# eridgd/WCT-TF

Measured on AMD Instinct MI355X. Metric: stylized frames/sec @512x512, 5-level relu5->1 pipeline, alpha=0.8, higher is better.
Workload: dtype f16

## Files before the change

wct_tf_amd/build.py:

```python
import hashlib
import os
import subprocess
import sys
from concurrent.futures import ThreadPoolExecutor

HERE = os.path.dirname(os.path.abspath(__file__))
CSRC = os.path.join(HERE, 'csrc')
LIB = os.path.join(HERE, 'libwct_hip.so')
WCT_UNITS = ['stats_gemm.hip', 'eigh.hip', 'spectral.hip', 'wct.hip', 'mask.hip', 'style_swap.hip', 'warm.hip']
API_UNITS = ['api_ctx.hip', 'api_weights.hip', 'api_drivers.hip', 'api_ops.hip', 'api_stylize.hip', 'api_train.hip']
SOURCES = API_UNITS + ['conv.hip', 'conv_wino.hip', 'coral.hip', 'colors.hip', 'guided.hip', 'guided_color.hip', 'guided_time.hip', 'guided_motion.hip', 'noise.hip', 'resize.hip', 'banded.hip', 'wrap.hip', 'train.hip'] + WCT_UNITS


STAMP = LIB + '.src.sha256'
FLAGS = ['--offload-arch=gfx950', '-O3', '-std=c++17', '-fPIC', '-Wno-unused-value', '-Wno-unused-result']
FILE_FLAGS = {u: ['-fno-slp-vectorize'] for u in WCT_UNITS}


def source_digest():
    h = hashlib.sha256((' '.join(FLAGS) + repr(sorted(FILE_FLAGS.items()))).encode())
    deps = sorted(os.path.join(CSRC, f) for f in os.listdir(CSRC) if f.endswith(('.hip', '.h')))
    deps.append(os.path.join(os.path.dirname(HERE), 'include', 'wct_hip.h'))
    for d in deps:
        h.update(os.path.basename(d).encode())
# ... 37 lines not shown
```

wct_tf_amd/csrc/banded.hip:

```cpp
#include "api.h"
#include "wct_stages.h"
#include "pool_rule.h"

static const int BAND_RE[6] = {0, 16, 16, 16, 48, 96};
static const int BAND_RD[6] = {0, 2, 2, 3, 4, 5};
constexpr int BAND_ROWS_CAP = 2048;
constexpr size_t LAUNCH_BYTES = WCT_LAUNCH_BYTES;

struct Band { int e0, e1, y0, y1, d0, d1, f0, f1; };

static void band_list(int H, int level, int band_rows, std::vector<Band>* out) {
  const int s = 1 << (level - 1), h = (H + s - 1) / s, Re = BAND_RE[level], Rd = BAND_RD[level];
  out->clear();
  for (long long y = 0; y < H; y += band_rows) {
    Band b;
    b.y0 = (int)y; b.y1 = (int)std::min<long long>(H, y + band_rows);
    b.e0 = std::max(0, b.y0 - Re); b.e1 = (int)std::min<long long>(H, (long long)b.y1 + Re);
    b.f0 = b.y0 / s; b.f1 = b.y1 == H ? h : b.y1 / s;
    b.d0 = std::max(0, b.f0 - Rd) & ~1; b.d1 = std::min(h, b.f1 + Rd);
    out->push_back(b);
  }
}

static bool enc_fits(long long rows, long long W, int level) {
// ... 334 lines not shown
      HIP_TRY(hipGetLastError());
      HIP_TRY(hipMemcpyAsync(cp.means + (size_t)k0 * C, gp.w.mean, (size_t)G * C * sizeof(float), hipMemcpyDeviceToDevice, s));
      HIP_TRY(hipMemcpyAsync(cp.scales + k0, gp.w.scale, (size_t)G * sizeof(float), hipMemcpyDeviceToDevice, s));
    }
    hipLaunchKernelGGL(pool_finish_kernel, dim3(C), dim3(C), 0, s, (const double*)cp.acc, (const float*)cp.means, (const float*)cp.scales,
                       (const int*)cp.n, K, C, cov_eps(mode, r.eps), w.mean, w.A, w.A0, w.scale);
    HIP_TRY(hipGetLastError());
  }
  if ((stages & WCT_STAGE_EIG) && (rc = launch_eig_stage(w, C, 1, cp.tail.skip, 1, r.sweeps_dev, r.eig_fail, s))) return rc;
  if (!(stages & WCT_STAGE_APPLY)) return WCT_OK;
  if (prep) {
    WctStyleSlots slots = {};
    slots.state[0] = prep->state[0];
    if ((rc = launch_style_load_slots(slots, 1, w, C, true, s))) return rc;
  }
  if ((rc = launch_spectral_tail(w, C, 1, r.alpha, mode, r.eps, cp.tail.skip, 1, s))) return rc;
  if ((rc = launch_blend(w, C, 1, r.alpha, cp.tail.skip, s))) return rc;
  for (int k = 0; k < K; ++k) {
    const size_t at = (size_t)k * n_full * C;
    if ((rc = launch_apply(w, content + at, k == K - 1 ? n_last : n_full, C, 1, r.out16 ? r.out16 + at : nullptr, r.out32 ? r.out32 + at : nullptr, s)))
      return rc;
  }
  return WCT_OK;
}

int run_transform_chunked(wct_ctx* c, const float* fc, size_t Nc, int n_full, int K, const float* fs, int Ns, int C, float alpha,
                          unsigned flags, float eps, half_t* out16, float* out32, int* sweeps_dev, const WctStyleRef* prep) {
  ARG_CHECK(K >= 1 && n_full >= 1 && Nc > (size_t)n_full * (K - 1) && Nc < LAUNCH_BYTES);
  if (flags & WCT_FLAG_ADAIN) { wct_set_error("a chunked transform is a whiten-colour transform: WCT_FLAG_ADAIN is not served"); return WCT_ERR_ARG; }
  if (K == 1) return run_transform(c, fc, (int)Nc, fs, Ns, C, 1, alpha, flags, eps, out16, out32, sweeps_dev, nullptr, prep);
  if (K > CHUNKS_MAX) { wct_set_error("%d chunks: at most %d per map", K, CHUNKS_MAX); return WCT_ERR_ARG; }
// ... 12 lines not shown
```

wct_tf_amd/csrc/mask.hip:

```cpp
#include "wct_stages.h"
#include <algorithm>
#include <type_traits>

constexpr int MASK_ROWS = 2048;
constexpr int SEG_STRIDE = WCT_MIX_MAX + 1;

__device__ __forceinline__ int mask_label(const MaskGeom& g, int r) {
  const int i = r / g.w, j = r - i * g.w;
  return g.mask[(size_t)min(i * g.stride, g.Hm - 1) * g.Wm + min(j * g.stride, g.Wm - 1)];
}

__global__ __launch_bounds__(256) void mask_count_kernel(MaskGeom g, int N, int K, int* counts) {
  __shared__ int wc[4][WCT_MIX_MAX];
  g.mask += (size_t)blockIdx.y * g.Hm * g.Wm;
  counts += (size_t)blockIdx.y * gridDim.x * WCT_MIX_MAX;
  const int lane = threadIdx.x & 63, wave = threadIdx.x >> 6;
  int cnt[WCT_MIX_MAX];
#pragma unroll
  for (int k = 0; k < WCT_MIX_MAX; ++k) cnt[k] = 0;
  const int base = blockIdx.x * MASK_ROWS;
  for (int it = 0; it < MASK_ROWS / 256; ++it) {
    const int r = base + it * 256 + threadIdx.x;
    const int lab = r < N ? mask_label(g, r) : -1;
#pragma unroll
// ... 217 lines not shown
  const int mode = r.mode, stages = r.stages; hipStream_t s = r.stream;
  MaskPlan m;
  ARG_CHECK(C % 32 == 0 && C >= 32 && C <= 1024 && content && styles && mask_plan(&m, r.workspace, C, Nc, nk, styles, Ns, K, 2));
  ARG_CHECK(mode == WCT_MODE_NP || mode == WCT_MODE_TF);
  ARG_CHECK(launch_map_fits((size_t)Nc * C, 4) && plan_fits(m, C));
  ARG_CHECK(r.workspace_bytes >= m.total);
  const WctCarve& w = m.w;
  int rc;
  if (stages & WCT_STAGE_COV) {
    if ((rc = launch_mask_gather(content, g, Nc, K, C, m, 1, s))) return rc;
    if ((rc = launch_plan_stats(m, C, false, true, cov_eps(mode, r.eps), s))) return rc;
  }
  if ((stages & WCT_STAGE_EIG) && m.P > 0 && (rc = launch_eig_stage(w, C, m.P, m.skip, 1, r.sweeps_dev, r.eig_fail, s))) return rc;
  if (!(stages & WCT_STAGE_APPLY)) return WCT_OK;
  if (m.P > 0) {
    if ((rc = launch_spectral_tail(w, C, m.P, r.alpha, mode, r.eps, m.skip, m.nwhite, s))) return rc;
    if ((rc = launch_blend(w, C, m.P, r.alpha, m.skip, s))) return rc;
    ApplySegArgs a = apply_args<ApplySegArgs>(w, m.xg, 0, C, r.out16, r.out32);
    a.seg_off = m.seg_off; a.perm = m.perm;
    for (int p = 0; p < WCT_MIX_MAX; ++p) a.lab[p] = m.lab[p];
    if ((rc = launch_apply_args(a, m.nmax, m.P, s))) return rc;
  }
  return launch_mask_passthrough(content, Nc, C, m, 1, K, r.out16, r.out32, s);
}

struct SegLabels { int lab[WCT_MIX_MAX]; };
struct SegBatchLabels { unsigned char fl[WCT_PLAN_PAIRS]; int N; };
template <typename Labels>
__global__ void adain_seg_apply_kernel(const float* xg, const int* seg_off, const int* perm, Labels sl, int C, const float* mean,
                                       const float* var, float alpha, float eps, half_t* out16, float* out32) {
  const int pair = blockIdx.y;
// ... 116 lines not shown
  ARG_CHECK(C % 32 == 0 && C >= 32 && C <= 1024 && content && mask_batch_plan(&m, r.workspace, C, Nc, G, nk, Ns, K, 2));
  ARG_CHECK(mode == WCT_MODE_NP || mode == WCT_MODE_TF);
  ARG_CHECK(launch_map_fits((size_t)Nc * C, 4) && plan_fits(m, C));
  ARG_CHECK((size_t)G * Nc < ((size_t)1 << 31));
  ARG_CHECK(r.workspace_bytes >= m.total);
  const WctCarve& w = m.w;
  int rc;
  if (stages & WCT_STAGE_COV) {
    if ((rc = launch_mask_gather(content, g, Nc, K, C, m, m.G, s))) return rc;
    if ((rc = launch_plan_stats(m, C, false, true, cov_eps(mode, r.eps), s))) return rc;
  }
  if ((stages & WCT_STAGE_EIG) && m.P > 0 && (rc = launch_eig_stage(w, C, m.P, m.skip, 1, nullptr, r.eig_fail, s))) return rc;
  if (!(stages & WCT_STAGE_APPLY)) return WCT_OK;
  if (m.P > 0) {
    if ((rc = launch_style_load_slots(states, m.P, w, C, true, s))) return rc;
    if ((rc = launch_spectral_tail(w, C, m.P, r.alpha, mode, r.eps, m.skip, m.nwhite, s))) return rc;
    if ((rc = launch_blend(w, C, m.P, r.alpha, m.skip, s))) return rc;
    ApplySegBatchArgs a = apply_args<ApplySegBatchArgs>(w, m.xg, Nc, C, r.out16, r.out32);
    a.seg_off = m.seg_off; a.perm = m.perm;
    for (int p = 0; p < WCT_PLAN_PAIRS; ++p) a.fl[p] = m.fl[p];
    if ((rc = launch_apply_args(a, m.nmax, m.P, s))) return rc;
  }
  return launch_mask_passthrough(content, Nc, C, m, m.G, K, r.out16, r.out32, s);
}

int launch_adain_masked_batch(const float* content, int Nc, int G, const MaskGeom& g, const int* nk, const int* Ns, int K, int C,
                              const WctCall& r, const WctStyleSlots& states) {
  hipStream_t s = r.stream;
  MaskBatchPlan m;
  ARG_CHECK(C % 32 == 0 && C <= 1024 && content && mask_batch_plan(&m, r.workspace, C, Nc, G, nk, Ns, K, 1));
  ARG_CHECK((size_t)G * Nc < ((size_t)1 << 31));
// ... 18 lines not shown
```

wct_tf_amd/csrc/spectral.hip:

```cpp
#include "wct_stages.h"

__device__ __forceinline__ bool pair_resolved(float dp, float dq, float e) { return e * e <= 0.25f * dp * dq; }

constexpr float SPECTRAL_NOISE_CUT = 2.f;
__device__ __forceinline__ float spectral_cut(const float* Am, int C, int tid, float* red) {
  float mn = 0.f;
  for (int i = tid; i < C; i += 256) mn = fminf(mn, Am[(size_t)i * C + i]);
  for (int o = 32; o > 0; o >>= 1) mn = fminf(mn, __shfl_xor(mn, o, 64));
  if ((tid & 63) == 0) red[tid >> 6] = mn;
  __syncthreads();
  mn = fminf(fminf(red[0], red[1]), fminf(red[2], red[3]));
  return fmaxf(1e-5f, -SPECTRAL_NOISE_CUT * mn);
}

__device__ __forceinline__ float spectral_entry(float dp, float dq, float e, bool diag, int kind, float shift, float cut) {
  const bool kp = dp > cut, kq = dq > cut;
  if (diag) return kp ? (kind == 0 ? 1.f / sqrtf(dp + shift) : sqrtf(dp + shift)) : 0.f;
  if (!kp && !kq) return 0.f;
  if (kp && kq) {
    if (!pair_resolved(dp, dq, e)) return 0.f;
    const float sa = sqrtf(dp + shift), sb = sqrtf(dq + shift);
    return kind == 0 ? -e / (sa * sb * (sa + sb)) : e / (sa + sb);
  }
  const float dk = kp ? dp : dq, dd = kp ? dq : dp;
// ... 13 lines not shown
  for (int i = 0; i < 4; ++i) {
    const int r = q0 + ty * 4 + i, c = p0 + tx * 4;
    f32x4 v = {0.f, 0.f, 0.f, 0.f};
    if (r < C && c < C) v = *reinterpret_cast<const f32x4*>(Am + (size_t)r * C + c);
#pragma unroll
    for (int j = 0; j < 4; ++j) t.mt[ty * 4 + i][tx * 4 + j] = v[j];
  }
}

struct SpecAllArgs {
  const float* A;
  float* G;
  float *N, *R, *Pm;
  const float *X1, *X2;
  int C; float shift; int correct, second; WctSkip skip;
  unsigned* mabs; const float* mean; float* bias; float alpha; int mode;
};

__global__ __launch_bounds__(256) void spectral_open_all_kernel(SpecAllArgs a) {
  __shared__ SpectralTile t;
  const int m = blockIdx.z, p0 = blockIdx.y * 64, q0 = blockIdx.x * 64, tid = threadIdx.x;
  const int C = a.C, kind = m & 1, pair = m >> 1;
  const size_t cc = (size_t)C * C;
  if (kind == 0 && blockIdx.x == 0 && blockIdx.y == 0) {
    if (tid == 0) a.mabs[pair] = 0u;
    const float* mp = a.mean + (size_t)(one_content(a.skip) ? 0 : pair) * 2 * C;
    const float* ms = a.mean + (size_t)(one_style(a.skip) ? 0 : pair) * 2 * C + C;
    for (int i = tid; i < C; i += 256) {
      float b = a.alpha * ms[i];
      if (a.mode == WCT_MODE_TF) b += (1.f - a.alpha) * mp[i];
      a.bias[pair * C + i] = b;
    }
// ... 14 lines not shown
    f32x4 g, n4 = {0.f, 0.f, 0.f, 0.f}, r4 = n4, p4 = n4;
#pragma unroll
    for (int j = 0; j < 4; ++j) {
      const float dk = t.dq[tx * 4 + j];
      const float em = 0.5f * (av[j] + t.mt[tx * 4 + j][pl]);
      g[j] = spectral_entry(dp, dk, a.correct ? em : 0.f, p == q + j, kind, a.shift, cut);
      if (a.second && p != q + j && dp > cut && dk > cut && pair_resolved(dp, dk, em)) {
        const float sp = sqrtf(dp + a.shift), sk = sqrtf(dk + a.shift);
        n4[j] = em / (sp + sk);
        r4[j] = em / sk;
        p4[j] = n4[j] / sk;
      }
    }
    const size_t o = (size_t)p * C + q;
    *reinterpret_cast<f32x4*>(a.G + m * cc + o) = g;
    if (a.second) {
      *reinterpret_cast<f32x4*>(a.N + m * cc + o) = n4;
      if (kind == 0) { *reinterpret_cast<f32x4*>(a.R + pair * cc + o) = r4; *reinterpret_cast<f32x4*>(a.Pm + pair * cc + o) = p4; }
    }
  }
}

__global__ __launch_bounds__(256) void spectral_add2_all_kernel(SpecAllArgs a) {
  __shared__ float dps[64], dqs[64];
  __shared__ float x1t[64][65], x2t[64][65];
  const int m = blockIdx.z, p0 = blockIdx.y * 64, q0 = blockIdx.x * 64, tid = threadIdx.x;
  if (skip_style_mat(m, a.skip)) return;
  const int C = a.C, kind = m & 1;
  const size_t cc = (size_t)C * C;
  const float* Am = a.A + m * cc;
  float* Gm = a.G + m * cc;
  const float* X2 = a.X2 + m * cc;
  const float* X1 = a.X1 + (size_t)(m >> 1) * cc;
  int near = 0;
  for (int i = tid; i < C; i += 256) {
    const float d = fabsf(Am[(size_t)i * C + i]);
    near |= (d > 3.3e-6f) & (d < 3e-5f);
  }
  if (__syncthreads_or(near)) return;
  __shared__ float cutred[4];
  const float cut = spectral_cut(Am, C, tid, cutred);
  if (tid < 64) dps[tid] = p0 + tid < C ? Am[(size_t)(p0 + tid) * C + p0 + tid] : 0.f;
  else if (tid < 128) dqs[tid - 64] = q0 + tid - 64 < C ? Am[(size_t)(q0 + tid - 64) * C + q0 + tid - 64] : 0.f;
  const int ty = tid >> 4, tx = tid & 15;
#pragma unroll
  for (int i = 0; i < 4; ++i) {
    const int r = q0 + ty * 4 + i, c = p0 + tx * 4;
    f32x4 v1 = {0.f, 0.f, 0.f, 0.f}, v2 = v1;
    if (r < C && c < C) {
      v2 = *reinterpret_cast<const f32x4*>(X2 + (size_t)r * C + c);
      if (kind == 0) v1 = *reinterpret_cast<const f32x4*>(X1 + (size_t)r * C + c);
    }
#pragma unroll
    for (int j = 0; j < 4; ++j) { x2t[ty * 4 + i][tx * 4 + j] = v2[j]; x1t[ty * 4 + i][tx * 4 + j] = v1[j]; }
  }
  __syncthreads();
#pragma unroll
  for (int i = 0; i < 4; ++i) {
    const int pl = ty * 4 + i, p = p0 + pl, q = q0 + tx * 4;
    if (p >= C || q >= C) continue;
    const size_t o = (size_t)p * C + q;
    const f32x4 x2 = *reinterpret_cast<const f32x4*>(X2 + o);
    f32x4 x1 = {0.f, 0.f, 0.f, 0.f};
    if (kind == 0) x1 = *reinterpret_cast<const f32x4*>(X1 + o);
    f32x4 g = *reinterpret_cast<const f32x4*>(Gm + o);
    const float dp = dps[pl];
#pragma unroll
    for (int j = 0; j < 4; ++j) {
      const float dq = dqs[tx * 4 + j];
      if (!(dp > cut && dq > cut)) continue;
      const float sp = sqrtf(dp + a.shift), sq = sqrtf(dq + a.shift);
      float l2;
      if (kind == 1) l2 = -0.5f * (x2[j] + x2t[tx * 4 + j][pl]) / (sp + sq);
      else l2 = (0.5f * (x1[j] + x1t[tx * 4 + j][pl]) + 0.25f * (sp + sq) * (x2[j] + x2t[tx * 4 + j][pl])) / (sp * sq * (sp + sq));
      g[j] += l2;
    }
    *reinterpret_cast<f32x4*>(Gm + o) = g;
  }
}

static GemmArgs level_product(int C, WctSkip skip) {
  GemmArgs g = {};
  g.lda = g.ldb = g.ldo = C; g.M = g.N = g.K = g.ksplit = C; g.sA = g.sB = g.s_out = (size_t)C * C; g.skip = skip;
  return g;
}

static int launch_refresh(const WctCarve& w, int C, int P, WctSkip skip, hipStream_t s) {
  int rc;
  GemmArgs r1 = level_product(C, skip);
  r1.A = w.A0; r1.a_kmajor = 0; r1.B = w.V; r1.b_kmajor = 1; r1.out32 = w.X;
  r1.mask_diag = w.A; r1.s_mask = (size_t)C * C; r1.mask_out = w.refresh;
  if ((rc = launch_gemm(r1, 1, 2 * P, s))) return rc;
  GemmArgs r2 = level_product(C, skip);
  r2.A = w.V; r2.a_kmajor = 1; r2.B = w.X; r2.b_kmajor = 1; r2.out32 = w.A; r2.mask_in = w.refresh;
  return launch_gemm(r2, 1, 2 * P, s);
}

int launch_spectral_tail_refreshed(const WctCarve& w, int C, int P, float alpha, int mode, float eps_in, WctSkip skip, int nwhite,
                                   hipStream_t s) {
  int rc;
  const size_t cc = (size_t)C * C;
  const float shift = mode == WCT_MODE_NP ? (eps_in >= 0.f ? eps_in : 1e-5f) : 0.f;
  const int second = EIG_CORRECT >= 2;
  const dim3 tiles(cdiv(C, 64), cdiv(C, 64), 2 * P);
  SpecAllArgs sa = {};
  sa.A = w.A; sa.G = w.G; sa.C = C; sa.shift = shift; sa.correct = EIG_CORRECT; sa.second = second; sa.skip = skip;
  sa.N = w.S2; float* X2 = sa.N + 2 * P * cc; sa.R = X2 + 2 * P * cc; sa.Pm = sa.R + P * cc; float* X1 = sa.Pm + P * cc;
  sa.X1 = X1; sa.X2 = X2;
  sa.mabs = w.mabs; sa.mean = w.mean; sa.bias = w.bias; sa.alpha = alpha; sa.mode = mode;
  hipLaunchKernelGGL(spectral_open_all_kernel, tiles, dim3(256), 0, s, sa);
  HIP_TRY(hipGetLastError());
  if (second) {
    GemmArgs a = level_product(C, skip);
    a.A = sa.Pm; a.A_odd = sa.N + cc; a.sA_odd = 2 * cc; a.a_kmajor = 0; a.B = sa.N; a.b_kmajor = 1; a.out32 = X2;
    if ((rc = launch_gemm(a, 1, 2 * P, s))) return rc;
    GemmArgs b = level_product(C, WCT_SKIP_NONE);
    b.A = sa.R; b.a_kmajor = 0; b.B = sa.N; b.b_kmajor = 1; b.sB = 2 * cc; b.out32 = X1;
    if (nwhite > 0 && (rc = launch_gemm(b, 1, nwhite, s))) return rc;
    hipLaunchKernelGGL(spectral_add2_all_kernel, tiles, dim3(256), 0, s, sa);
    HIP_TRY(hipGetLastError());
  }
  GemmArgs g = level_product(C, skip);
  g.A = w.V; g.a_kmajor = 0; g.B = w.G; g.b_kmajor = 1; g.out32 = w.X;
  if ((rc = launch_gemm(g, 1, 2 * P, s))) return rc;
  GemmArgs h = level_product(C, skip);
  h.A = w.X; h.a_kmajor = 0; h.B = w.V; h.b_kmajor = 0; h.out32 = w.Tw;
  return launch_gemm(h, 1, 2 * P, s);
}

int launch_spectral_tail(const WctCarve& w, int C, int P, float alpha, int mode, float eps_in, WctSkip skip, int nwhite,
                         hipStream_t s) {
  const int rc = launch_refresh(w, C, P, skip, s);
  return rc ? rc : launch_spectral_tail_refreshed(w, C, P, alpha, mode, eps_in, skip, nwhite, s);
}
```

wct_tf_amd/csrc/style_swap.hip:

```cpp
#include "wct_stages.h"

__global__ void im2col_kernel(const float* src, float* dst, int w, int C, int p, int st, int ho, int wo) {
  const int c4n = C / 4;
  const size_t total = (size_t)ho * wo * p * p * c4n;
  for (size_t e = blockIdx.x * (size_t)blockDim.x + threadIdx.x; e < total; e += (size_t)gridDim.x * blockDim.x) {
    const int c4 = (int)(e % c4n);
    size_t t = e / c4n;
    const int j = (int)(t % p); t /= p;
    const int i = (int)(t % p); t /= p;
    const int x = (int)(t % wo), y = (int)(t / wo);
    reinterpret_cast<f32x4*>(dst)[e] =
        *reinterpret_cast<const f32x4*>(src + ((size_t)(y * st + i) * w + (x * st + j)) * C + c4 * 4);
  }
}

__global__ void patch_axis_inv_norm_kernel(const float* B, float* inv, int n, int K) {
  const int k4 = blockIdx.x * blockDim.x + threadIdx.x;
  if (k4 * 4 >= K) return;
  f32x4 s = {0.f, 0.f, 0.f, 0.f};
  for (int r = 0; r < n; ++r) {
    const f32x4 v = *reinterpret_cast<const f32x4*>(B + (size_t)r * K + k4 * 4);
    s += v * v;
  }
  f32x4 o;
// ... 111 lines not shown
                  "(swap_filter_fit / center_crop_to, wct.py:84-90)", patch, stride, hc, wc,
                  (ho - 1) * stride + patch, (wo - 1) * stride + patch);
    return WCT_ERR_ARG;
  }
  const int Nc = hc * wc, Ns = hs * ws, Mo = ho * wo, Pn = rows * cols, K = patch * patch * C;
  const size_t wct_bytes = align_up(wct_workspace_bytes(C, Nc, Ns, 1));
  ARG_CHECK(workspace_bytes >= style_swap_workspace_bytes(C, hc, wc, hs, ws, patch, stride));
  WctCarve w = carve(workspace, C, 1, pair_layout(C, Nc, Ns));
  SwapCarve sw = swap_carve((char*)workspace + wct_bytes, C, hc, wc, hs, ws, patch, stride);
  int rc;
  WctCall r = {};
  r.alpha = alpha; r.mode = WCT_MODE_TF; r.eps = eps; r.workspace = workspace; r.workspace_bytes = wct_bytes;
  r.stages = WCT_STAGE_COV | WCT_STAGE_EIG | WCT_STAGE_EIG_FP32UPDATE; r.eig_fail = eig_fail; r.stream = s;
  if ((rc = launch_wct(content, Nc, style, Ns, C, 1, WCT_SKIP_NONE, r, nullptr, nullptr, nullptr))) return rc;
  const size_t cc = (size_t)C * C;
  if ((rc = launch_spectral_tail(w, C, 1, alpha, WCT_MODE_TF, eps, WCT_SKIP_NONE, 1, s))) return rc;
  WctCarve v = w;
  v.A += cc; v.V += cc; v.G += cc; v.X += cc; v.Tw = w.T;
  if ((rc = launch_spectral_tail_refreshed(v, C, 1, alpha, WCT_MODE_TF, eps, WCT_SKIP_STYLE, 1, s))) return rc;
  auto apply = [&](const float* X, int N, const float* mean, const float* T, float* out) {
    GemmArgs g = {};
    g.A = X; g.lda = C; g.a_kmajor = 0; g.a_sub_k = mean; g.B = T; g.ldb = C; g.b_kmajor = 0;
    g.M = N; g.N = C; g.K = C; g.ksplit = C; g.out32 = out; g.ldo = C;
    return launch_gemm(g, 1, 1, s);
  };
  if ((rc = apply(content, Nc, w.mean, w.Tw, sw.Wc))) return rc;
  if ((rc = apply(style, Ns, w.mean + C, w.T, sw.Ws))) return rc;
  hipLaunchKernelGGL(im2col_kernel, dim3(ew_grid((size_t)Mo * K / 4)), dim3(256), 0, s, sw.Wc, sw.Ac, wc, C, patch, stride, ho, wo);
  hipLaunchKernelGGL(im2col_kernel, dim3(ew_grid((size_t)Pn * K / 4)), dim3(256), 0, s, sw.Ws, sw.Bs, ws, C, patch, stride, rows, cols);
  hipLaunchKernelGGL(patch_axis_inv_norm_kernel, dim3(cdiv(K / 4, 64)), dim3(64), 0, s, sw.Bs, sw.inv, Pn, K);
  HIP_TRY(hipGetLastError());
  {
    GemmArgs g = {};
    g.A = sw.Ac; g.lda = K; g.a_kmajor = 0; g.a_scale_k = sw.inv; g.B = sw.Bs; g.ldb = K; g.b_kmajor = 0;
// ... 20 lines not shown
```

wct_tf_amd/csrc/wct.hip:

```cpp
#include "wct_stages.h"
#include "jacobi_dev.h"
#include "strength_rule.h"
#include "conv_first_tile.h"
#include <algorithm>
#include <type_traits>



template <int BC, int BP, typename Args = ApplyArgs>
__global__ __launch_bounds__(256, 2) void apply_f16x2_kernel(Args p) {
  constexpr bool SEGB = std::is_same<Args, ApplySegBatchArgs>::value;
  constexpr bool SEG = std::is_same<Args, ApplySegArgs>::value || SEGB;
  constexpr bool MAP = std::is_same<Args, ApplyMapArgs>::value;
  constexpr int TM = BC / 64, TN = BP / 64;
  constexpr int MI = BC * 4 / 256, XI = BP * 4 / 256;
  __shared__ __attribute__((aligned(16))) unsigned char lm[2][BC * 64];
  __shared__ __attribute__((aligned(16))) unsigned char lx[2][BP * 64];
  typedef unsigned int u32x4 __attribute__((ext_vector_type(4)));
  const int tid = threadIdx.x, lane = tid & 63, wave = tid >> 6;
  const int wm = wave >> 1, wn = wave & 1;
  const int pair = blockIdx.z;
  const int n0 = blockIdx.x * BP, c0 = blockIdx.y * BC;
  int seg0 = 0, N = p.N;
  [[maybe_unused]] int row0 = 0;
// ... 511 lines not shown
  ARG_CHECK(style && state && C % 32 == 0 && C >= 32 && C <= 1024 && Ns >= (adain ? 1 : 2) && launch_map_fits((size_t)Ns * C, 4));
  ARG_CHECK(adain || mode == WCT_MODE_NP || mode == WCT_MODE_TF);
  ARG_CHECK(key.nslab >= 1 && key.nslab <= 256 && key.nsplit >= 1 && key.ksplit >= 256 && key.ksplit % 32 == 0 &&
            (long long)key.nsplit * key.ksplit >= Ns);
  SlotPlan sp;
  style_plan(&sp, r.workspace, C, style, Ns, key);
  ARG_CHECK(r.workspace_bytes >= sp.total);
  const WctCarve& w = sp.w;
  int rc;
  if (adain) {
    if ((rc = launch_plan_stats(sp, C, true, false, 0.f, s))) return rc;
    HIP_TRY(hipMemcpyAsync(state + C, w.var + C, (size_t)C * sizeof(float), hipMemcpyDeviceToDevice, s));
  } else {
    if ((rc = launch_plan_stats(sp, C, false, true, cov_eps(mode, r.eps), s))) return rc;
    if ((rc = launch_eig_stage(w, C, sp.P, sp.skip, 1, nullptr, r.eig_fail, s))) return rc;
    if ((rc = launch_spectral_tail(w, C, sp.P, 1.f, mode, r.eps, sp.skip, sp.nwhite, s))) return rc;
    HIP_TRY(hipMemcpyAsync(state + 2 * C, w.Tw + (size_t)C * C, (size_t)C * C * sizeof(float), hipMemcpyDeviceToDevice, s));
  }
  HIP_TRY(hipMemcpyAsync(state, w.mean + C, (size_t)C * sizeof(float), hipMemcpyDeviceToDevice, s));
  return WCT_OK;
}

int launch_wct(const float* content, int Nc, const float* style, int Ns, int C, int P, WctSkip skip, const WctCall& r,
               const WctFeatStats* stats, const WctStyleRef* prep, const WctWarmRef* warm, const WctStrength* sm, const WctImageSrc* src) {
  const int mode = r.mode, stages = r.stages; hipStream_t s = r.stream;
  ARG_CHECK(C % 32 == 0 && C >= 32 && C <= 1024 && Nc >= 2 && Ns >= 2 && P >= 1 && P <= 32);
  ARG_CHECK(!src || (C == 64 && !prep && !warm && !sm && stats && stats->u[0] && stats->umax[0] && stats->u[1] && stats->umax[1] &&
                     src->side[0].H * src->side[0].W == Nc && src->side[1].H * src->side[1].W == Ns));
  ARG_CHECK(!sm || strength_ok(*sm, Nc));
  ARG_CHECK(skip == WCT_SKIP_NONE || skip == WCT_SKIP_SHARED_STYLE);
  ARG_CHECK(!warm || (warm->basis && (skip == WCT_SKIP_NONE || prep)));
// ... 8 lines not shown
    if (src) rc = launch_cov_image(*src, P, w, cov_eps(mode, r.eps), skip, s);
    else rc = launch_cov(content, Nc, style, Ns, C, P, w, cov_eps(mode, r.eps), skip, s);
    if (rc) return rc;
  }
  if (stages & WCT_STAGE_EIG) {
    const bool rotate = warm && warm->valid;
    if (rotate && (rc = launch_warm_rotate(w, C, P, warm->basis, s))) return rc;
    if ((rc = launch_eig_stage(w, C, P, skip, (stages & WCT_STAGE_EIG_FP32UPDATE) ? 0 : 1, r.sweeps_dev, r.eig_fail, s, rotate ? 0 : 2)))
      return rc;
    if (rotate && (rc = launch_warm_compose(w, C, P, warm->basis, s))) return rc;
    if (warm && (rc = launch_warm_store(w.V + (size_t)2 * (P - 1) * C * C, w.X, warm->basis, C, s))) return rc;
  }
  if (!(stages & WCT_STAGE_APPLY)) return WCT_OK;

  if (prep && (rc = launch_style_load(*prep, 1, w, C, true, s))) return rc;
  if ((rc = launch_spectral_tail(w, C, P, sm ? 1.f : r.alpha, mode, r.eps, skip, P, s))) return rc;
  if (sm) return launch_blend_apply_map(w, content, Nc, C, P, skip, r, *sm);
  if (src) {
    if ((rc = launch_blend(w, C, P, r.alpha, skip, s))) return rc;
    return launch_apply_image(w, *src, P, r.out16, r.out32, s);
  }
  return launch_blend_apply(w, content, Nc, C, P, skip, r);
}

void plan_carve(SlotPlan* sp, void* base, int C) {
  PairLayout mx = {1, 1, 0};
  for (int m = 0; m < 2 * sp->P; ++m)
    if (sp->slot[m].n) { mx.nslab = std::max(mx.nslab, sp->slot[m].lay.nslab); mx.nsplit = std::max(mx.nsplit, sp->slot[m].lay.nsplit); }
  sp->w = carve(base, C, std::max(sp->P, 1), mx);
  sp->total = sp->w.total;
}
// ... 55 lines not shown
int launch_wct_mix(const float* content, int Nc, const float* const* styles, const int* Ns, int K, const float* lambda, int C,
                   const WctCall& r, const WctFeatStats* stats, const WctStyleRef* prep) {
  const int mode = r.mode, stages = r.stages; hipStream_t s = r.stream;
  SlotPlan sp;
  ARG_CHECK(C % 32 == 0 && C >= 32 && C <= 1024 && Nc >= 2 && content && (styles || prep) &&
            mix_plan(&sp, r.workspace, C, content, Nc, prep ? nullptr : styles, Ns, K, lambda, 2, stats, prep != nullptr));
  ARG_CHECK(mode == WCT_MODE_NP || mode == WCT_MODE_TF);
  ARG_CHECK(plan_fits(sp, C));
  ARG_CHECK(r.workspace_bytes >= sp.total);
  const WctCarve& w = sp.w;
  int rc;
  if ((stages & WCT_STAGE_COV) && (rc = launch_plan_stats(sp, C, false, true, cov_eps(mode, r.eps), s))) return rc;
  if ((stages & WCT_STAGE_EIG) && (rc = launch_eig_stage(w, C, sp.P, sp.skip, 1, r.sweeps_dev, r.eig_fail, s))) return rc;
  if (!(stages & WCT_STAGE_APPLY)) return WCT_OK;
  if (prep && (rc = launch_style_load(*prep, K, w, C, true, s))) return rc;
  if ((rc = launch_spectral_tail(w, C, sp.P, r.alpha, mode, r.eps, sp.skip, sp.nwhite, s))) return rc;
  MixWeights mw = {};
  mw.K = K;
  for (int k = 0; k < K; ++k) mw.lambda[k] = lambda[k];
  const size_t n4 = (size_t)C * C / 4;
  hipLaunchKernelGGL(wct_mix_kernel, dim3((unsigned)std::min<size_t>((n4 + 255) / 256, 1024)), dim3(256), 0, s, w.Tw, w.bias, C, mw);
  HIP_TRY(hipGetLastError());
  return launch_blend_apply(w, content, Nc, C, 1, WCT_SKIP_NONE, r);
}

__global__ void adain_apply_kernel(const float* x, size_t n4_per_pair, int C, const float* mean, const float* var,
                                   float alpha, float eps, half_t* out16, float* out32, int style_of_pair0,
                                   const float* mix_mu = nullptr, const float* mix_sd = nullptr) {
  const int pair = blockIdx.y;
  const int cq = C / 4;
  const float* mp = mean + (size_t)pair * 2 * C;
// ... 116 lines not shown
```

wct_tf_amd/csrc/wct_stages.h:

```cpp
#pragma once
#include "common.h"


constexpr int EIG_CORRECT = 2;
constexpr float JACOBI_TOL_FN = 1.5e-2f;
constexpr float JACOBI_TOL_FN2 = 4e-2f;
constexpr float JACOBI_TOL_FN_WCT = EIG_CORRECT >= 2 ? JACOBI_TOL_FN2 : (EIG_CORRECT ? JACOBI_TOL_FN : 0.f);

static inline size_t align_up(size_t x) { return (x + 255) & ~(size_t)255; }

struct WctCarve {
  float *mean, *var, *stat_partial, *absmax, *scale, *cov_partial, *A, *A0, *V, *d, *G, *X, *S2, *Tw, *Tcs, *T, *M, *bias, *mix;
  unsigned* mabs; int* refresh;
  void* jacobi_ws; size_t jacobi_bytes;
  int nslab, nsplit, ksplit;
  size_t total;
};

struct PairLayout { int nslab, nsplit, ksplit; };
PairLayout pair_layout(int C, int Nc, int Ns);
WctCarve carve(void* base, int C, int P, const PairLayout& lay);

static inline float cov_eps(int mode, float eps_in) {
  return mode == WCT_MODE_TF ? (eps_in >= 0.f ? eps_in : 1e-8f) : 0.f;
// ... 32 lines not shown
  a.x = x; a.N = N; a.C = C; a.mean = w.mean; a.M = w.M; a.bias = w.bias;
  a.xscale = w.scale; a.mabs = w.mabs; a.out16 = out16; a.out32 = out32;
  return a;
}
__device__ __host__ __forceinline__ int seg_frame(unsigned char fl) { return fl >> 3; }
__device__ __host__ __forceinline__ int seg_label(unsigned char fl) { return fl & 7; }

int launch_means(const float* content, int Nc, const float* style, int Ns, int C, int P, const WctCarve& w, bool with_var,
                 WctSkip skip, hipStream_t s, const WctFeatStats* fs);
int launch_cov(const float* content, int Nc, const float* style, int Ns, int C, int P, const WctCarve& w, float eps, WctSkip skip,
               hipStream_t s);
int launch_plan_stats(const SlotPlan& sp, int C, bool with_var, bool with_cov, float eps, hipStream_t s);
int launch_cov_image(const WctImageSrc& src, int P, const WctCarve& w, float eps, WctSkip skip, hipStream_t s);
int launch_eig_stage(const WctCarve& w, int C, int P, WctSkip skip, int u_f16, int* sweeps_dev, int* eig_fail, hipStream_t s,
                     int check_from = 2);
int launch_spectral_tail(const WctCarve& w, int C, int P, float alpha, int mode, float eps_in, WctSkip skip, int nwhite, hipStream_t s);
int launch_spectral_tail_refreshed(const WctCarve& w, int C, int P, float alpha, int mode, float eps_in, WctSkip skip, int nwhite,
                                   hipStream_t s);
int launch_blend(const WctCarve& w, int C, int P, float alpha, WctSkip skip, hipStream_t s);
int launch_apply(const WctCarve& w, const float* content, int Nc, int C, int P, half_t* out16, float* out32, hipStream_t s);
template <typename Args> int launch_apply_args(const Args& a, int nmax, int P, hipStream_t s);
int launch_warm_rotate(const WctCarve& w, int C, int P, const float* V0, hipStream_t s);
int launch_warm_compose(const WctCarve& w, int C, int P, const float* V0, hipStream_t s);
int launch_warm_store(const float* V, float* scratch, float* basis, int C, hipStream_t s);
int launch_style_load_slots(const WctStyleSlots& r, int P, const WctCarve& w, int C, bool with_T, hipStream_t s);
```

Before: 698.3.

## Run second-order spectral products as split-bf16 MFMA GEMMs with upper-triangle tiles

In the spectral tail, the second-order correction matrices are stored as hi/lo bf16 planes and multiplied by a new MFMA kernel that uses three bf16 products to approximate fp32 accuracy. The symmetric X2 product computes only upper-triangular tiles, and the add kernel reads the mirrored half to reconstruct the full matrix. This is meant to replace the fp32 GEMM path with cheaper matrix-core work and roughly halve the symmetric product. It costs some precision and adds a new kernel, and it is enabled by default with an environment variable to fall back to fp32.

```diff
diff --git a/wct_tf_amd/build.py b/wct_tf_amd/build.py
--- a/wct_tf_amd/build.py
+++ b/wct_tf_amd/build.py
@@ -7,7 +7,7 @@
 HERE = os.path.dirname(os.path.abspath(__file__))
 CSRC = os.path.join(HERE, 'csrc')
 LIB = os.path.join(HERE, 'libwct_hip.so')
-WCT_UNITS = ['stats_gemm.hip', 'eigh.hip', 'spectral.hip', 'wct.hip', 'mask.hip', 'style_swap.hip', 'warm.hip']
+WCT_UNITS = ['stats_gemm.hip', 'eigh.hip', 'spectral.hip', 'spectral_gemm.hip', 'wct.hip', 'mask.hip', 'style_swap.hip', 'warm.hip']
 API_UNITS = ['api_ctx.hip', 'api_weights.hip', 'api_drivers.hip', 'api_ops.hip', 'api_stylize.hip', 'api_train.hip']
 SOURCES = API_UNITS + ['conv.hip', 'conv_wino.hip', 'coral.hip', 'colors.hip', 'guided.hip', 'guided_color.hip', 'guided_time.hip', 'guided_motion.hip', 'noise.hip', 'resize.hip', 'banded.hip', 'wrap.hip', 'train.hip'] + WCT_UNITS
 
diff --git a/wct_tf_amd/csrc/banded.hip b/wct_tf_amd/csrc/banded.hip
--- a/wct_tf_amd/csrc/banded.hip
+++ b/wct_tf_amd/csrc/banded.hip
@@ -372,7 +372,7 @@
     slots.state[0] = prep->state[0];
     if ((rc = launch_style_load_slots(slots, 1, w, C, true, s))) return rc;
   }
-  if ((rc = launch_spectral_tail(w, C, 1, r.alpha, mode, r.eps, cp.tail.skip, 1, s))) return rc;
+  if ((rc = launch_spectral_tail(w, C, 1, r.alpha, mode, r.eps, cp.tail.skip, 1, second_order_bf16(), s))) return rc;
   if ((rc = launch_blend(w, C, 1, r.alpha, cp.tail.skip, s))) return rc;
   for (int k = 0; k < K; ++k) {
     const size_t at = (size_t)k * n_full * C;
diff --git a/wct_tf_amd/csrc/mask.hip b/wct_tf_amd/csrc/mask.hip
--- a/wct_tf_amd/csrc/mask.hip
+++ b/wct_tf_amd/csrc/mask.hip
@@ -255,7 +255,7 @@
   if ((stages & WCT_STAGE_EIG) && m.P > 0 && (rc = launch_eig_stage(w, C, m.P, m.skip, 1, r.sweeps_dev, r.eig_fail, s))) return rc;
   if (!(stages & WCT_STAGE_APPLY)) return WCT_OK;
   if (m.P > 0) {
-    if ((rc = launch_spectral_tail(w, C, m.P, r.alpha, mode, r.eps, m.skip, m.nwhite, s))) return rc;
+    if ((rc = launch_spectral_tail(w, C, m.P, r.alpha, mode, r.eps, m.skip, m.nwhite, second_order_bf16(), s))) return rc;
     if ((rc = launch_blend(w, C, m.P, r.alpha, m.skip, s))) return rc;
     ApplySegArgs a = apply_args<ApplySegArgs>(w, m.xg, 0, C, r.out16, r.out32);
     a.seg_off = m.seg_off; a.perm = m.perm;
@@ -402,7 +402,7 @@
   if (!(stages & WCT_STAGE_APPLY)) return WCT_OK;
   if (m.P > 0) {
     if ((rc = launch_style_load_slots(states, m.P, w, C, true, s))) return rc;
-    if ((rc = launch_spectral_tail(w, C, m.P, r.alpha, mode, r.eps, m.skip, m.nwhite, s))) return rc;
+    if ((rc = launch_spectral_tail(w, C, m.P, r.alpha, mode, r.eps, m.skip, m.nwhite, second_order_bf16(), s))) return rc;
     if ((rc = launch_blend(w, C, m.P, r.alpha, m.skip, s))) return rc;
     ApplySegBatchArgs a = apply_args<ApplySegBatchArgs>(w, m.xg, Nc, C, r.out16, r.out32);
     a.seg_off = m.seg_off; a.perm = m.perm;
diff --git a/wct_tf_amd/csrc/spectral.hip b/wct_tf_amd/csrc/spectral.hip
--- a/wct_tf_amd/csrc/spectral.hip
+++ b/wct_tf_amd/csrc/spectral.hip
@@ -51,8 +51,18 @@
   float *N, *R, *Pm;
   const float *X1, *X2;
   int C; float shift; int correct, second; WctSkip skip;
+  int split;
   unsigned* mabs; const float* mean; float* bias; float alpha; int mode;
 };
+
+__device__ __forceinline__ void split_bf16_store(float* mat, size_t cc, size_t o, f32x4 v) {
+  bf16x4 h, l;
+#pragma unroll
+  for (int j = 0; j < 4; ++j) { h[j] = (bf16_t)v[j]; l[j] = (bf16_t)(v[j] - (float)h[j]); }
+  bf16_t* planes = reinterpret_cast<bf16_t*>(mat);
+  *reinterpret_cast<bf16x4*>(planes + o) = h;
+  *reinterpret_cast<bf16x4*>(planes + cc + o) = l;
+}
 
 __global__ __launch_bounds__(256) void spectral_open_all_kernel(SpecAllArgs a) {
   __shared__ SpectralTile t;
@@ -97,7 +107,10 @@
     }
     const size_t o = (size_t)p * C + q;
     *reinterpret_cast<f32x4*>(a.G + m * cc + o) = g;
-    if (a.second) {
+    if (a.second && a.split) {
+      split_bf16_store(a.N + m * cc, cc, o, n4);
+      if (kind == 0) { split_bf16_store(a.R + pair * cc, cc, o, r4); split_bf16_store(a.Pm + pair * cc, cc, o, p4); }
+    } else if (a.second) {
       *reinterpret_cast<f32x4*>(a.N + m * cc + o) = n4;
       if (kind == 0) { *reinterpret_cast<f32x4*>(a.R + pair * cc + o) = r4; *reinterpret_cast<f32x4*>(a.Pm + pair * cc + o) = p4; }
     }
@@ -126,12 +139,13 @@
   if (tid < 64) dps[tid] = p0 + tid < C ? Am[(size_t)(p0 + tid) * C + p0 + tid] : 0.f;
   else if (tid < 128) dqs[tid - 64] = q0 + tid - 64 < C ? Am[(size_t)(q0 + tid - 64) * C + q0 + tid - 64] : 0.f;
   const int ty = tid >> 4, tx = tid & 15;
+  const bool above = a.split && p0 < q0, below = a.split && p0 > q0;
 #pragma unroll
   for (int i = 0; i < 4; ++i) {
     const int r = q0 + ty * 4 + i, c = p0 + tx * 4;
     f32x4 v1 = {0.f, 0.f, 0.f, 0.f}, v2 = v1;
     if (r < C && c < C) {
-      v2 = *reinterpret_cast<const f32x4*>(X2 + (size_t)r * C + c);
+      if (!above) v2 = *reinterpret_cast<const f32x4*>(X2 + (size_t)r * C + c);
       if (kind == 0) v1 = *reinterpret_cast<const f32x4*>(X1 + (size_t)r * C + c);
     }
 #pragma unroll
@@ -143,7 +157,8 @@
     const int pl = ty * 4 + i, p = p0 + pl, q = q0 + tx * 4;
     if (p >= C || q >= C) continue;
     const size_t o = (size_t)p * C + q;
-    const f32x4 x2 = *reinterpret_cast<const f32x4*>(X2 + o);
+    f32x4 x2 = {0.f, 0.f, 0.f, 0.f};
+    if (!below) x2 = *reinterpret_cast<const f32x4*>(X2 + o);
     f32x4 x1 = {0.f, 0.f, 0.f, 0.f};
     if (kind == 0) x1 = *reinterpret_cast<const f32x4*>(X1 + o);
     f32x4 g = *reinterpret_cast<const f32x4*>(Gm + o);
@@ -154,8 +169,9 @@
       if (!(dp > cut && dq > cut)) continue;
       const float sp = sqrtf(dp + a.shift), sq = sqrtf(dq + a.shift);
       float l2;
-      if (kind == 1) l2 = -0.5f * (x2[j] + x2t[tx * 4 + j][pl]) / (sp + sq);
-      else l2 = (0.5f * (x1[j] + x1t[tx * 4 + j][pl]) + 0.25f * (sp + sq) * (x2[j] + x2t[tx * 4 + j][pl])) / (sp * sq * (sp + sq));
+      const float x2m = above ? x2[j] : x2t[tx * 4 + j][pl], x2d = below ? x2m : x2[j];
+      if (kind == 1) l2 = -0.5f * (x2d + x2m) / (sp + sq);
+      else l2 = (0.5f * (x1[j] + x1t[tx * 4 + j][pl]) + 0.25f * (sp + sq) * (x2d + x2m)) / (sp * sq * (sp + sq));
       g[j] += l2;
     }
     *reinterpret_cast<f32x4*>(Gm + o) = g;
@@ -180,7 +196,7 @@
 }
 
 int launch_spectral_tail_refreshed(const WctCarve& w, int C, int P, float alpha, int mode, float eps_in, WctSkip skip, int nwhite,
-                                   hipStream_t s) {
+                                   int second_bf16, hipStream_t s) {
   int rc;
   const size_t cc = (size_t)C * C;
   const float shift = mode == WCT_MODE_NP ? (eps_in >= 0.f ? eps_in : 1e-5f) : 0.f;
@@ -188,12 +204,26 @@
   const dim3 tiles(cdiv(C, 64), cdiv(C, 64), 2 * P);
   SpecAllArgs sa = {};
   sa.A = w.A; sa.G = w.G; sa.C = C; sa.shift = shift; sa.correct = EIG_CORRECT; sa.second = second; sa.skip = skip;
+  sa.split = second && second_bf16 && C % 64 == 0;
   sa.N = w.S2; float* X2 = sa.N + 2 * P * cc; sa.R = X2 + 2 * P * cc; sa.Pm = sa.R + P * cc; float* X1 = sa.Pm + P * cc;
   sa.X1 = X1; sa.X2 = X2;
   sa.mabs = w.mabs; sa.mean = w.mean; sa.bias = w.bias; sa.alpha = alpha; sa.mode = mode;
   hipLaunchKernelGGL(spectral_open_all_kernel, tiles, dim3(256), 0, s, sa);
   HIP_TRY(hipGetLastError());
-  if (second) {
+  if (sa.split) {
+    const size_t mat = 2 * cc;
+    const bf16_t* Nb = reinterpret_cast<const bf16_t*>(sa.N);
+    Prod2Args a = {};
+    a.A = reinterpret_cast<const bf16_t*>(sa.Pm); a.sA = mat; a.A_odd = Nb + mat; a.sA_odd = 2 * mat; a.B = Nb; a.sB = mat;
+    a.out = X2; a.s_out = cc; a.C = C; a.upper = 1; a.skip = skip;
+    if ((rc = launch_prod_bf16x2(a, 2 * P, s))) return rc;
+    Prod2Args b = {};
+    b.A = reinterpret_cast<const bf16_t*>(sa.R); b.sA = mat; b.B = Nb; b.sB = 2 * mat;
+    b.out = X1; b.s_out = cc; b.C = C; b.upper = 0; b.skip = WCT_SKIP_NONE;
+    if (nwhite > 0 && (rc = launch_prod_bf16x2(b, nwhite, s))) return rc;
+    hipLaunchKernelGGL(spectral_add2_all_kernel, tiles, dim3(256), 0, s, sa);
+    HIP_TRY(hipGetLastError());
+  } else if (second) {
     GemmArgs a = level_product(C, skip);
     a.A = sa.Pm; a.A_odd = sa.N + cc; a.sA_odd = 2 * cc; a.a_kmajor = 0; a.B = sa.N; a.b_kmajor = 1; a.out32 = X2;
     if ((rc = launch_gemm(a, 1, 2 * P, s))) return rc;
@@ -212,7 +242,12 @@
 }
 
 int launch_spectral_tail(const WctCarve& w, int C, int P, float alpha, int mode, float eps_in, WctSkip skip, int nwhite,
-                         hipStream_t s) {
+                         int second_bf16, hipStream_t s) {
   const int rc = launch_refresh(w, C, P, skip, s);
-  return rc ? rc : launch_spectral_tail_refreshed(w, C, P, alpha, mode, eps_in, skip, nwhite, s);
-}
+  return rc ? rc : launch_spectral_tail_refreshed(w, C, P, alpha, mode, eps_in, skip, nwhite, second_bf16, s);
+}
+
+int second_order_bf16() {
+  static const int f32 = getenv("WCT_SECOND_ORDER_F32") ? atoi(getenv("WCT_SECOND_ORDER_F32")) : 0;
+  return !f32;
+}
diff --git a/wct_tf_amd/csrc/spectral_gemm.hip b/wct_tf_amd/csrc/spectral_gemm.hip
--- /dev/null
+++ b/wct_tf_amd/csrc/spectral_gemm.hip
@@ -0,0 +1,119 @@
+#include "wct_stages.h"
+
+template <int BT>
+__global__ __launch_bounds__(256, 2) void prod_bf16x2_kernel(Prod2Args p) {
+  constexpr int TM = BT / 64;
+  __shared__ __attribute__((aligned(16))) unsigned char lds[4][BT * 64];
+  const int tid = threadIdx.x, lane = tid & 63, wave = tid >> 6;
+  const int wm = wave >> 1, wn = wave & 1;
+  int ti, tj;
+  if (p.upper) {
+    ti = 0; int rem = blockIdx.x;
+    while (rem >= p.ntile - ti) { rem -= p.ntile - ti; ++ti; }
+    tj = ti + rem;
+  } else {
+    ti = blockIdx.x / p.ntile; tj = blockIdx.x % p.ntile;
+  }
+  const int m0 = ti * BT, n0 = tj * BT;
+  const int batch = blockIdx.z, C = p.C;
+  if (skip_style_mat(batch, p.skip)) return;
+  const size_t cc = (size_t)C * C;
+  const bf16_t* A = p.A_odd ? ((batch & 1) ? p.A_odd + (batch >> 1) * p.sA_odd : p.A + (batch >> 1) * p.sA) : p.A + batch * p.sA;
+  const bf16_t* B = p.B + batch * p.sB;
+
+  f32x16 acc[TM][TM];
+#pragma unroll
+  for (int i = 0; i < TM; ++i)
+#pragma unroll
+    for (int j = 0; j < TM; ++j)
+#pragma unroll
+      for (int r = 0; r < 16; ++r) acc[i][j][r] = 0.f;
+
+  bf16x8 ra[2][TM], rb[2][TM];
+  auto load = [&](int k0) {
+#pragma unroll
+    for (int i = 0; i < TM; ++i) {
+      const int id = tid + i * 256, row = id >> 2, chunk = id & 3;
+      const size_t oa = (size_t)(m0 + row) * C + k0 + chunk * 8, ob = (size_t)(n0 + row) * C + k0 + chunk * 8;
+      ra[0][i] = *reinterpret_cast<const bf16x8*>(A + oa);
+      ra[1][i] = *reinterpret_cast<const bf16x8*>(A + cc + oa);
+      rb[0][i] = *reinterpret_cast<const bf16x8*>(B + ob);
+      rb[1][i] = *reinterpret_cast<const bf16x8*>(B + cc + ob);
+    }
+  };
+  auto park = [&]() {
+#pragma unroll
+    for (int i = 0; i < TM; ++i) {
+      const int id = tid + i * 256, row = id >> 2, chunk = id & 3;
+      const int off = (row * 4 + (chunk ^ ((row >> 2) & 3))) * 16;
+      *reinterpret_cast<bf16x8*>(lds[0] + off) = ra[0][i];
+      *reinterpret_cast<bf16x8*>(lds[1] + off) = ra[1][i];
+      *reinterpret_cast<bf16x8*>(lds[2] + off) = rb[0][i];
+      *reinterpret_cast<bf16x8*>(lds[3] + off) = rb[1][i];
+    }
+  };
+
+  load(0);
+  for (int k0 = 0; k0 < C; k0 += 32) {
+    park();
+    __syncthreads();
+    if (k0 + 32 < C) load(k0 + 32);
+#pragma unroll
+    for (int ks = 0; ks < 2; ++ks) {
+      const int chunk = ks * 2 + (lane >> 5);
+      bf16x8 ah[TM], al[TM], bh[TM], bl[TM];
+#pragma unroll
+      for (int i = 0; i < TM; ++i) {
+        const int r = (wm * TM + i) * 32 + (lane & 31);
+        const int off = (r * 4 + (chunk ^ ((r >> 2) & 3))) * 16;
+        ah[i] = *reinterpret_cast<const bf16x8*>(lds[0] + off);
+        al[i] = *reinterpret_cast<const bf16x8*>(lds[1] + off);
+      }
+#pragma unroll
+      for (int j = 0; j < TM; ++j) {
+        const int r = (wn * TM + j) * 32 + (lane & 31);
+        const int off = (r * 4 + (chunk ^ ((r >> 2) & 3))) * 16;
+        bh[j] = *reinterpret_cast<const bf16x8*>(lds[2] + off);
+        bl[j] = *reinterpret_cast<const bf16x8*>(lds[3] + off);
+      }
+#pragma unroll
+      for (int i = 0; i < TM; ++i)
+#pragma unroll
+        for (int j = 0; j < TM; ++j) {
+          acc[i][j] = __builtin_amdgcn_mfma_f32_32x32x16_bf16(ah[i], bl[j], acc[i][j], 0, 0, 0);
+          acc[i][j] = __builtin_amdgcn_mfma_f32_32x32x16_bf16(al[i], bh[j], acc[i][j], 0, 0, 0);
+          acc[i][j] = __builtin_amdgcn_mfma_f32_32x32x16_bf16(ah[i], bh[j], acc[i][j], 0, 0, 0);
+        }
+    }
+    __syncthreads();
+  }
+
+  float* out = p.out + batch * p.s_out;
+#pragma unroll
+  for (int i = 0; i < TM; ++i)
+#pragma unroll
+    for (int j = 0; j < TM; ++j) {
+      const int gm0 = m0 + (wm * TM + i) * 32, gn = n0 + (wn * TM + j) * 32 + (lane & 31);
+      if (p.upper && (gm0 >> 6) > (gn >> 6)) continue;
+#pragma unroll
+      for (int r = 0; r < 16; ++r) {
+        const int gm = gm0 + (r & 3) + 8 * (r >> 2) + 4 * (lane >> 5);
+        out[(size_t)gm * C + gn] = acc[i][j][r];
+      }
+    }
+}
+
+int launch_prod_bf16x2(Prod2Args a, int nbatch, hipStream_t s) {
+  if (a.C % 64) return WCT_ERR_ARG;
+  const long big = a.upper ? (long)(a.C / 128) * (a.C / 128 + 1) / 2 : (long)(a.C / 128) * (a.C / 128);
+  if (a.C % 128 == 0 && big * nbatch >= 256) {
+    a.ntile = a.C / 128;
+    hipLaunchKernelGGL((prod_bf16x2_kernel<128>), dim3((unsigned)big, 1, nbatch), dim3(256), 0, s, a);
+  } else {
+    a.ntile = a.C / 64;
+    const unsigned nblk = a.upper ? a.ntile * (a.ntile + 1) / 2 : a.ntile * a.ntile;
+    hipLaunchKernelGGL((prod_bf16x2_kernel<64>), dim3(nblk, 1, nbatch), dim3(256), 0, s, a);
+  }
+  HIP_TRY(hipGetLastError());
+  return WCT_OK;
+}
diff --git a/wct_tf_amd/csrc/style_swap.hip b/wct_tf_amd/csrc/style_swap.hip
--- a/wct_tf_amd/csrc/style_swap.hip
+++ b/wct_tf_amd/csrc/style_swap.hip
@@ -149,10 +149,10 @@
   r.stages = WCT_STAGE_COV | WCT_STAGE_EIG | WCT_STAGE_EIG_FP32UPDATE; r.eig_fail = eig_fail; r.stream = s;
   if ((rc = launch_wct(content, Nc, style, Ns, C, 1, WCT_SKIP_NONE, r, nullptr, nullptr, nullptr))) return rc;
   const size_t cc = (size_t)C * C;
-  if ((rc = launch_spectral_tail(w, C, 1, alpha, WCT_MODE_TF, eps, WCT_SKIP_NONE, 1, s))) return rc;
+  if ((rc = launch_spectral_tail(w, C, 1, alpha, WCT_MODE_TF, eps, WCT_SKIP_NONE, 1, 0, s))) return rc;
   WctCarve v = w;
   v.A += cc; v.V += cc; v.G += cc; v.X += cc; v.Tw = w.T;
-  if ((rc = launch_spectral_tail_refreshed(v, C, 1, alpha, WCT_MODE_TF, eps, WCT_SKIP_STYLE, 1, s))) return rc;
+  if ((rc = launch_spectral_tail_refreshed(v, C, 1, alpha, WCT_MODE_TF, eps, WCT_SKIP_STYLE, 1, 0, s))) return rc;
   auto apply = [&](const float* X, int N, const float* mean, const float* T, float* out) {
     GemmArgs g = {};
     g.A = X; g.lda = C; g.a_kmajor = 0; g.a_sub_k = mean; g.B = T; g.ldb = C; g.b_kmajor = 0;
diff --git a/wct_tf_amd/csrc/wct.hip b/wct_tf_amd/csrc/wct.hip
--- a/wct_tf_amd/csrc/wct.hip
+++ b/wct_tf_amd/csrc/wct.hip
@@ -549,7 +549,7 @@
   } else {
     if ((rc = launch_plan_stats(sp, C, false, true, cov_eps(mode, r.eps), s))) return rc;
     if ((rc = launch_eig_stage(w, C, sp.P, sp.skip, 1, nullptr, r.eig_fail, s))) return rc;
-    if ((rc = launch_spectral_tail(w, C, sp.P, 1.f, mode, r.eps, sp.skip, sp.nwhite, s))) return rc;
+    if ((rc = launch_spectral_tail(w, C, sp.P, 1.f, mode, r.eps, sp.skip, sp.nwhite, second_order_bf16(), s))) return rc;
     HIP_TRY(hipMemcpyAsync(state + 2 * C, w.Tw + (size_t)C * C, (size_t)C * C * sizeof(float), hipMemcpyDeviceToDevice, s));
   }
   HIP_TRY(hipMemcpyAsync(state, w.mean + C, (size_t)C * sizeof(float), hipMemcpyDeviceToDevice, s));
@@ -588,7 +588,7 @@
   if (!(stages & WCT_STAGE_APPLY)) return WCT_OK;
 
   if (prep && (rc = launch_style_load(*prep, 1, w, C, true, s))) return rc;
-  if ((rc = launch_spectral_tail(w, C, P, sm ? 1.f : r.alpha, mode, r.eps, skip, P, s))) return rc;
+  if ((rc = launch_spectral_tail(w, C, P, sm ? 1.f : r.alpha, mode, r.eps, skip, P, second_order_bf16(), s))) return rc;
   if (sm) return launch_blend_apply_map(w, content, Nc, C, P, skip, r, *sm);
   if (src) {
     if ((rc = launch_blend(w, C, P, r.alpha, skip, s))) return rc;
@@ -674,7 +674,7 @@
   if ((stages & WCT_STAGE_EIG) && (rc = launch_eig_stage(w, C, sp.P, sp.skip, 1, r.sweeps_dev, r.eig_fail, s))) return rc;
   if (!(stages & WCT_STAGE_APPLY)) return WCT_OK;
   if (prep && (rc = launch_style_load(*prep, K, w, C, true, s))) return rc;
-  if ((rc = launch_spectral_tail(w, C, sp.P, r.alpha, mode, r.eps, sp.skip, sp.nwhite, s))) return rc;
+  if ((rc = launch_spectral_tail(w, C, sp.P, r.alpha, mode, r.eps, sp.skip, sp.nwhite, second_order_bf16(), s))) return rc;
   MixWeights mw = {};
   mw.K = K;
   for (int k = 0; k < K; ++k) mw.lambda[k] = lambda[k];
diff --git a/wct_tf_amd/csrc/wct_stages.h b/wct_tf_amd/csrc/wct_stages.h
--- a/wct_tf_amd/csrc/wct_stages.h
+++ b/wct_tf_amd/csrc/wct_stages.h
@@ -70,9 +70,22 @@
 int launch_cov_image(const WctImageSrc& src, int P, const WctCarve& w, float eps, WctSkip skip, hipStream_t s);
 int launch_eig_stage(const WctCarve& w, int C, int P, WctSkip skip, int u_f16, int* sweeps_dev, int* eig_fail, hipStream_t s,
                      int check_from = 2);
-int launch_spectral_tail(const WctCarve& w, int C, int P, float alpha, int mode, float eps_in, WctSkip skip, int nwhite, hipStream_t s);
+int launch_spectral_tail(const WctCarve& w, int C, int P, float alpha, int mode, float eps_in, WctSkip skip, int nwhite,
+                         int second_bf16, hipStream_t s);
 int launch_spectral_tail_refreshed(const WctCarve& w, int C, int P, float alpha, int mode, float eps_in, WctSkip skip, int nwhite,
-                                   hipStream_t s);
+                                   int second_bf16, hipStream_t s);
+int second_order_bf16();
+typedef __bf16 bf16_t;
+typedef __bf16 bf16x4 __attribute__((ext_vector_type(4)));
+typedef __bf16 bf16x8 __attribute__((ext_vector_type(8)));
+struct Prod2Args {
+  const bf16_t* A; size_t sA;
+  const bf16_t* A_odd; size_t sA_odd;
+  const bf16_t* B; size_t sB;
+  float* out; size_t s_out;
+  int C, upper, ntile; WctSkip skip;
+};
+int launch_prod_bf16x2(Prod2Args a, int nbatch, hipStream_t s);
 int launch_blend(const WctCarve& w, int C, int P, float alpha, WctSkip skip, hipStream_t s);
 int launch_apply(const WctCarve& w, const float* content, int Nc, int C, int P, half_t* out16, float* out32, hipStream_t s);
 template <typename Args> int launch_apply_args(const Args& a, int nmax, int P, hipStream_t s);
```

Result: no change. 705.0 (median of 6 runs) (+1.0%).
